# codyheiser/MILWRM

Hardware: AMD Instinct MI355X
Metric: pixels/sec (node) for preprocess+k-means fit+label, 30-ch MxIF k=8; %HBM peak (higher is better)
Workload: dtype f32 (fp64 accumulation)

## Files before the change

### include/milwrm_amd.h

```cpp
#ifndef MILWRM_AMD_H
#define MILWRM_AMD_H

#include <stddef.h>
#include <stdint.h>

#ifdef __cplusplus
extern "C" {
#endif

#define MW_OK 0
#define MW_EINVAL (-1)
#define MW_EHIP (-2)
#define MW_EUNSUPPORTED (-3)

#define MW_U8 0
#define MW_U16 1
#define MW_F32 2

int mw_version(void);
const char* mw_last_error(void);
int mw_stream_blocks(int64_t n);
int64_t mw_rows_per_block(int64_t n);

size_t mw_nz_stats_ws_bytes(int64_t n_pix, int C);
// ... 39 lines not shown
                     void* d_ws, void* stream);
size_t mw_image_moments_rows_ws_bytes(int64_t slide_H);
int mw_image_moments_rows(const void* d_img, int dtype, int H, int W, int C,
                          int64_t row_off, int64_t slide_H, int pass,
                          const float* d_inv_mean, float pseudoval, void* d_ws, void* stream);
int mw_image_moments_rows_final(int64_t slide_H, int W, int C, int with_m2,
                                void* d_ws, double* d_out, void* stream);

size_t mw_blur_ws_bytes(int H, int W, int C, int radius);
int mw_blur(const void* d_img, int dtype, int H, int W, int C,
            const float* d_inv_mean, float pseudoval,
            const float* h_w, int radius, float* d_out, void* d_ws, void* stream);

int mw_block_mean(const void* d_img, int dtype, int H, int W, int C, int fact,
                  float* d_out, void* stream);

size_t mw_mask_rank_ws_bytes(int64_t n_pix);
int mw_mask_rank(const uint8_t* d_mask, int64_t n_pix, uint32_t* d_rank2pix,
                 int64_t* d_count, void* d_ws, void* stream);

size_t mw_rank_index_bytes(int64_t n_pix);
int mw_mask_rank_index(const uint8_t* d_mask, int64_t n_pix, void* d_index, int64_t* d_count, void* d_ws,
                       void* stream);

size_t mw_gather_ws_bytes(int64_t S, int F);
int mw_gather_rows(const float* d_img, int C, const int32_t* d_feat, int F,
                   const int32_t* d_idx, const uint32_t* d_rank2pix, int64_t S,
                   float* d_X, void* d_ws, void* stream);
int mw_gather_rows_ri(const float* d_img, int C, const int32_t* d_feat, int F, const int32_t* d_idx,
                      const void* d_index, int64_t n_pix, int64_t pix_off, int64_t S, float* d_X, void* d_ws,
                      void* stream);
int mw_rank_to_pixel_ri(int32_t* d_idx, int64_t S, const void* d_index, int64_t n_pix, int64_t pix_off,
                        void* stream);
int mw_gather_rows_px(const float* d_img, int C, const int32_t* d_feat, int F, const int32_t* d_pix, int64_t S,
                      float* d_X, void* d_ws, void* stream);
int mw_col_stats_rows(const float* d_X, int64_t S, int F, void* d_ws, void* stream);

size_t mw_sample_slot_elems(int64_t n_pix);
int mw_sample_map(const int32_t* d_idx, const uint32_t* d_rank2pix, int64_t S, int64_t n_pix,
                  int32_t* d_slots, int32_t* d_ovf, void* stream);
int mw_blur_sample(const void* d_img, int dtype, int H, int W, int C, const float* d_inv_mean,
                   float pseudoval, const float* h_weights, int radius, const int32_t* d_slots,
                   int64_t S, const int32_t* d_feat, int F, float* d_X, void* stream);
int mw_sample_overflow(const int32_t* d_idx, const uint32_t* d_rank2pix, const int32_t* d_slots,
                       const int32_t* d_ovf, int64_t S, int F, float* d_X, void* stream);
int mw_sample_map_ri(const int32_t* d_idx, const void* d_index, int64_t n_index, int64_t pix_off, int64_t S,
// ... 199 lines not shown
```

### milwrm_amd/MILWRM.py

```python
from __future__ import annotations

import itertools
import os

import numpy as np
import pandas as pd
import torch

from . import _native as N
from . import device as D
from .assign import (DOM_REC, assign_image, assign_rows, banded_assign_image, blur_assign_image,
                     dm_total, dom_carry_, dom_sums, domain_means, domain_sse_deferred, domain_sse_image,
                     domain_sse_rows, LabelPassQC)
from .kmeans import DeviceRows, KMeans, StandardScaler, fit_many
from .MxIF import checktype, img
from .ST import blur_features_st
from .dist import LOCAL_COMM
from .rng import _release_last_draw, check_total, set_global_state_after_draws, subsample_indices_device
from .stream import band_filter



def kMeansRes(scaled_data, k, alpha_k=0.02, random_state=18, comm=None):
    comm = LOCAL_COMM if comm is None else comm
# ... 205 lines not shown
                                      image._mask_device(), out_rows=out_rows, qc=q)
        if res is None and how != "fused" and fusable:
            res = blur_assign_image(raw, sigma, inv_mean, p, mu, inv, centers, image._mask_device(),
                                    truncate=truncate)
            q = None
        if res is not None:
            return out(res)
    elif image._pending_median is not None or image._pending_bilateral is not None:
        res = banded_assign_image(image._source() or image._device(), band_filter(image), feats, mu, inv,
                                  centers, image._mask_device(), qc=q)
        if res is not None:
            return out(res)
    src = D.as_float32(image._materialize())
    if band is not None:
        return out(assign_image(src[band.rows], feats, mu, inv, centers,
                                D.padded_mask(image._mask_device()[band.rows].contiguous())))
    res = assign_image(src, feats, mu, inv, centers, image._mask_device())
    if q is not None:
        q.band(src, res[0])
    return out(res)


_SIDE = {}
GATHER_BY_PIXEL = os.environ.get("MW_GATHER_PX", "0") == "1"
DRAWS_BESIDE = os.environ.get("MW_DRAWS_BESIDE", "1") != "0"


def _draws_beside(M: int, fract: float, dev, after: torch.cuda.Event, index=None):
    main = torch.cuda.current_stream(dev)
    side = _SIDE.get(str(dev))
    if side is None:
        side = _SIDE[str(dev)] = torch.cuda.Stream(device=dev)
    side.wait_event(after)
    with torch.cuda.stream(side):
        idx, tot = subsample_indices_device(M, fract, 16, dev)
        if index is not None:
            D.rank_to_pixel(idx, index)
    main.wait_stream(side)
    idx.record_stream(main)
    tot.record_stream(main)
    return idx, tot


def _gather_deferred(image: img, feat, idx, r2p, X_out) -> bool:
    from .stream import bilateral_gather, blur_gather, median_gather

    if image._pending_median is not None:
        inv_mean, p = image._pending if image._pending is not None else (None, 1.0)
        return median_gather(image._source() or image._device(), image._pending_median, inv_mean, p, feat,
                             idx, r2p, X_out)
    if image._pending_bilateral is not None:
        inv_mean, p = image._pending if image._pending is not None else (None, 1.0)
        return bilateral_gather(image._source() or image._device(), image._pending_bilateral, inv_mean, p, feat,
                                idx, r2p, X_out)
    if image._pending_blur is None:
        return False
    sigma, truncate = image._pending_blur
    inv_mean, p = image._pending
    return blur_gather(image._source() or image._device(), sigma, inv_mean, p, feat, idx, r2p, X_out,
                       truncate=truncate)
# ... 199 lines not shown
            if filter_kwargs is not None:
                raise NotImplementedError("filter_kwargs on a slide in row bands: the banded pass "
                                          "runs the gaussian only")
            X, img_stats, xmax = prep_banded(images[0], self.image_df["batch_names"].iloc[0],
                                             means, features, filter_name, sigma, fract, comm)
            self._batch_counts = [int(X.shape[0])]
            self._images = images
            st = comm.merge_image_stats(D.d2h(img_stats), X.shape[1])
            self.scaler = StandardScaler.from_stats(st)
            mu, inv = self.scaler.affine()
            self._rows = DeviceRows(X, mu, inv, feature_var=self.scaler.var_ * inv * inv,
                                    xmax_local=D.d2h(xmax))
            self._cluster_host = None
            return
        batches = list(self.image_df["batch_names"])
        ev0 = torch.cuda.Event()
        ev0.record()
        if images:
            images[0].log_normalize(mean=means[batches[0]])
            images[0].blurring(filter_name=filter_name, sigma=sigma, **fkw)
        dev = D.device()
        ranks = []
        for i, im in enumerate(images):
            r2p, M = im._mask_rank()
            ranks.append((r2p if i == 0 else None, M))
        counts = [int(M * fract) for _, M in ranks]
        F = len(images[0]._features(features))
        _check_rows_fit(sum(counts), F, dev)
        X = torch.empty((sum(counts), F), dtype=torch.float32, device=dev)
        img_stats = torch.zeros((len(images), 1 + 2 * F), dtype=torch.float64, device=dev)
        xmax = torch.zeros(F, dtype=torch.float32, device=dev)
        def by_pixel(im, r2p):
            return isinstance(r2p, D.RankIndex) and not im._filter_deferred() and GATHER_BY_PIXEL

        pre = None
        if images and counts[0] and DRAWS_BESIDE and not images[0]._filter_deferred():
            px0 = by_pixel(images[0], ranks[0][0])
            pre = _draws_beside(ranks[0][1], fract, dev, ev0, ranks[0][0] if px0 else None) + (px0,)
        off = 0
        paths = []
        totals = []
        draws = []
        moments = []
        rank_base = 0
        for n_img, (im, batch, (r2p, M), S) in enumerate(
                zip(images, self.image_df["batch_names"], ranks, counts)):
            if n_img > 0:
                im.log_normalize(mean=means[batch])
                im.blurring(filter_name=filter_name, sigma=sigma, **fkw)
            np.random.seed(16)
            if S:
                if r2p is None:
                    r2p, _ = im._mask_rank()
                if n_img == 0 and pre is not None:
                    idx, tot, px = pre
                    pre = None
                else:
                    idx, tot = subsample_indices_device(M, fract, 16, dev)
                    px = by_pixel(im, r2p)
                    if px:
                        D.rank_to_pixel(idx, r2p)
                totals.append((tot, S))
                feat = D.h2d(np.asarray(im._features(features), dtype=np.int32), dev)
                if _gather_deferred(im, feat, idx, r2p, X[off:off + S]):
                    rec = D.col_stats_rows(X[off:off + S], img_stats[n_img], accumulate=False,
                                           absmax=xmax, keep_records=True)
                else:
                    rec = D.gather_rows(D.as_float32(im._materialize()), feat, idx, None if px else r2p,
                                        X[off:off + S], img_stats[n_img], accumulate=False, absmax=xmax,
                                        keep_records=True)
                moments.append((off, S) + rec)
                draws.append((off, S, idx, rank_base))
                del idx
            else:
                _release_last_draw()
            r2p = None
            ranks[n_img] = (None, M)
            off += S
            rank_base += int(im.shape[0]) * int(im.shape[1])
            if use_path:
                paths.append(_save_preprocessed(im, self.image_df["Img"].iloc[n_img], path_save))
        self._batch_counts = counts
        if use_path:
            self.image_df["Img"] = paths
        else:
            self._images = images
        set_global_state_after_draws()
        host = D.d2h(img_stats, xmax, *[t for t, _ in totals])
        for (_, S), tot in zip(totals, host[2:]):
            check_total(int(tot[0]), S)
        st = comm.merge_image_stats(host[0], F)
# ... 274 lines not shown
```

### milwrm_amd/MxIF.py

```python
from __future__ import annotations

import os

import numpy as np
import torch

from . import device as D
from .rng import check_total, set_global_state_after_draws, subsample_indices_device


def checktype(obj):
    return bool(obj) and all(isinstance(elem, str) for elem in obj)


def _out_of_scope(name):
    def f(*a, **k):
        raise NotImplementedError(f"{name} is outside the MI355X hot path (plotting); use the reference "
                                  "implementation")
    f.__name__ = name
    return f


def _need_kernel_size(name):
    return NotImplementedError(f"{name}: pass kernel_size= (an int, a (rows, cols) pair, or None for an eighth "
# ... 300 lines not shown
        return (self._pending_blur is not None or self._pending_median is not None
                or self._pending_bilateral is not None)

    @property
    def mask(self):
        return self._mask

    @mask.setter
    def mask(self, m):
        self._mask = m
        self._mask_dev = None
        self._mrank = None

    def _mask_device(self) -> torch.Tensor:
        if self._mask_dev is None:
            if self._mask is None:
                raise AssertionError("No tissue mask available")
            m = np.ascontiguousarray(np.asarray(self._mask) != 0, dtype=np.uint8)
            self._mask_dev = D.padded_mask(torch.from_numpy(m).to(D.device()))
        return self._mask_dev

    def _prefetch_mask_rank(self):
        if getattr(self, "_mrank", None) is None and self._mask is not None:
            self._mrank = D.mask_rank_async(self._mask_device().reshape(-1))

    def _mask_rank(self):
        pending = getattr(self, "_mrank", None)
        self._mrank = None
        return D.mask_rank(self._mask_device().reshape(-1), pending)

    def __repr__(self) -> str:
        descr = "img object with {} of {} and shape {}px x {}px\n".format(
            np.ndarray, np.dtype("float64"), self.shape[0], self.shape[1]
        ) + "{} image channels:\n\t{}".format(self.n_ch, self.ch)
        if self.mask is not None:
            descr += "\n\ntissue mask {} of {} and shape {}px x {}px".format(
                type(self.mask), self.mask.dtype, self.mask.shape[0], self.mask.shape[1])
        return descr

    def copy(self) -> "img":
        new = img.__new__(img)
        new.__dict__.update(self.__dict__)
        new.ch = list(self.ch)
        new._host = None if self._host is None else self._host.copy()
        new._host64 = None if self._host64 is None else self._host64.copy()
        new._dev = None if self._dev is None else self._dev.clone()
        new._hsrc = None
        new._mask = None if self._mask is None else self._mask.copy()
        new._mask_dev = None
        new._mrank = None
        return new

# ... 341 lines not shown
            print("mean calculated to perform log normalization")
            s, _ = self._nz_stats()
            n = self.shape[0] * self.shape[1]
            mean = s.cpu().numpy() / n
        elif self._pending is not None or self._pending_blur is not None or self._pending_bilateral is not None:
            self._materialize()
        mean = np.asarray(mean, dtype=np.float64)
        with np.errstate(divide="ignore"):
            inv = (1.0 / mean).astype(np.float32)
        raw = self._raw_int_max() is not None and self._pending is None and self._pending_blur is None
        self._pending = (D.h2d(inv, D.device()), float(pseudoval))
        self._lognorm_host = (inv, float(pseudoval)) if raw else None
        self._xbound = None
        self._host64 = None

    def _subsample_device(self, features, fract=0.2, random_state=16, X_out=None, stats=None,
                          accumulate=False):
        from .stream import bilateral_gather, blur_gather, median_gather

        features = self._features(features)
        np.random.seed(random_state)
        deferred = self._filter_deferred()
        src = None if deferred else D.as_float32(self._materialize())
        r2p, M = self._mask_rank()
        dev = D.device()
        d_idx, total = subsample_indices_device(M, fract, random_state, dev)
        S = d_idx.shape[0]
        if X_out is None:
            X_out = torch.empty((S, len(features)), dtype=torch.float32, device=dev)
        if stats is None:
            stats = torch.zeros(1 + 2 * len(features), dtype=torch.float64, device=dev)
        if S:
            feat = D.h2d(np.asarray(features, dtype=np.int32), dev)
            if deferred:
                inv, p = self._pending if self._pending is not None else (None, 1.0)
                if self._pending_median is not None:
                    median_gather(self._source() or self._device(), self._pending_median, inv, p, feat,
                                  d_idx, r2p, X_out)
                elif self._pending_bilateral is not None:
                    bilateral_gather(self._source() or self._device(), self._pending_bilateral, inv, p, feat,
                                     d_idx, r2p, X_out)
                else:
                    sigma, truncate = self._pending_blur
                    blur_gather(self._source() or self._device(), sigma, inv, p, feat, d_idx, r2p, X_out,
                                truncate)
                D.col_stats_rows(X_out, stats, accumulate)
            else:
# ... 76 lines not shown
```

### milwrm_amd/_native.py

```python
from __future__ import annotations

import ctypes as C
import os
import threading

import torch

_HERE = os.path.dirname(os.path.abspath(__file__))
LIB_PATH = os.environ.get("MW_LIB") or os.path.join(_HERE, "libmilwrm_amd.so")

MW_U8, MW_U16, MW_F32 = 0, 1, 2
_EINVAL, _EHIP, _EUNSUP = -1, -2, -3

_lib = None
_lock = threading.Lock()

c_i64, c_i32, c_u32, c_u64 = C.c_int64, C.c_int, C.c_uint32, C.c_uint64
c_f32, c_sz, c_vp = C.c_float, C.c_size_t, C.c_void_p
c_dp = C.POINTER(C.c_double)

_PROTOS = {
    "mw_version": (c_i32, []),
    "mw_host_labels_f64": (c_i32, [c_vp, c_i64, c_vp, c_i32]),
    "mw_host_f32_to_f64": (c_i32, [c_vp, c_i64, c_vp, c_i32]),
# ... 91 lines not shown
    "mw_domain_sse": (c_i32, [c_vp, c_i32, c_vp, c_i32, c_vp, c_vp, c_vp, c_vp, c_vp, c_i32, c_i32, c_vp,
                              c_i64, c_vp, c_i32, c_vp, c_vp]),
    "mw_domain_sse_f64": (c_i32, [c_vp, c_i32, c_vp, c_i32, c_vp, c_vp, c_vp, c_vp, c_vp, c_i32, c_i32, c_vp,
                                  c_i64, c_vp, c_i32, c_vp, c_vp]),
    "mw_neighbor_mean": (c_i32, [c_vp, c_vp, c_i64, c_vp, c_i32, c_vp, c_vp]),
    "mw_col_stats_rows": (c_i32, [c_vp, c_i64, c_i32, c_vp, c_vp]),
    "mw_col_stats_absmax": (c_i32, [c_vp, c_i64, c_i32, c_vp, c_i32, c_vp]),
    "mw_sample_slot_elems": (c_sz, [c_i64]),
    "mw_sample_map": (c_i32, [c_vp, c_vp, c_i64, c_i64, c_vp, c_vp, c_vp]),
    "mw_blur_sample": (c_i32, [c_vp, c_i32, c_i32, c_i32, c_i32, c_vp, c_f32, c_vp, c_i32, c_vp, c_i64, c_vp, c_i32, c_vp, c_vp]),
    "mw_sample_overflow": (c_i32, [c_vp, c_vp, c_vp, c_vp, c_i64, c_i32, c_vp, c_vp]),
    "mw_blur_assign_conf": (c_i32, [c_vp, c_i32, c_i32, c_i32, c_i32, c_vp, c_f32, c_vp, c_i32, c_vp, c_vp, c_vp, c_i32, c_vp, c_vp, c_vp, c_vp]),
    "mw_domain_records": (c_i32, [c_vp, c_vp, c_i64, c_i32, c_i32, c_vp, c_vp]),
    "mw_synth_slide": (c_i32, [c_i32, c_i32, c_i32, c_vp, c_i32, c_vp, c_i32, c_i32, c_i32, c_u64, c_vp, c_vp, c_vp]),
    "mw_synth_rows": (c_i32, [c_i32, c_i32, c_i32, c_i32, c_i32, c_vp, c_i32, c_vp, c_i32, c_i32, c_i32, c_u64,
                              c_vp, c_vp, c_vp]),
    "mw_blur_sample_rows": (c_i32, [c_vp, c_i32, c_i32, c_i32, c_i32, c_i64, c_i32, c_i32, c_vp, c_f32, c_vp,
                                    c_i32, c_vp, c_i64, c_vp, c_i32, c_vp, c_vp]),
    "mw_rank_index_bytes": (c_sz, [c_i64]),
    "mw_mask_rank_index": (c_i32, [c_vp, c_i64, c_vp, c_vp, c_vp, c_vp]),
    "mw_gather_rows_ri": (c_i32, [c_vp, c_i32, c_vp, c_i32, c_vp, c_vp, c_i64, c_i64, c_i64, c_vp, c_vp, c_vp]),
    "mw_rank_to_pixel_ri": (c_i32, [c_vp, c_i64, c_vp, c_i64, c_i64, c_vp]),
    "mw_gather_rows_px": (c_i32, [c_vp, c_i32, c_vp, c_i32, c_vp, c_i64, c_vp, c_vp, c_vp]),
    "mw_sample_map_ri": (c_i32, [c_vp, c_vp, c_i64, c_i64, c_i64, c_i64, c_vp, c_vp, c_vp]),
    "mw_sample_overflow_ri": (c_i32, [c_vp, c_vp, c_i64, c_i64, c_vp, c_vp, c_i64, c_i32, c_vp, c_vp]),
    "mw_slot_gather": (c_i32, [c_vp, c_i32, c_i64, c_i64, c_vp, c_i64, c_vp, c_i32, c_vp, c_vp]),
    "mw_blur_assign_rows": (c_i32, [c_vp, c_i32, c_i32, c_i32, c_i32, c_i64, c_i32, c_i32, c_vp, c_f32, c_vp,
                                    c_i32, c_vp, c_vp, c_vp, c_i32, c_vp, c_vp, c_vp, c_vp]),
}

EXPORTED = tuple(_PROTOS)


class LloydFit(C.Structure):
    _fields_ = [("centers", c_vp), ("drift", c_vp), ("half_sep", c_vp), ("labels", c_vp),
                ("ub", c_vp), ("lb", c_vp), ("ws", c_vp), ("out", c_vp), ("k", c_i32),
                ("drift_max", c_f32), ("inertia_exp", c_i32)]


class KppSeg(C.Structure):
    _fields_ = [("row_start", c_i64), ("n_rows", c_i64), ("rows_per_block", c_i64), ("d_records", c_vp)]


ALL_REDUCE_SUM_FN = C.CFUNCTYPE(c_i32, c_vp, c_i64, c_i64, c_vp)
ALL_GATHER_FN = C.CFUNCTYPE(c_i32, c_vp, c_i64, c_i64, c_i64, c_vp)

# ... 62 lines not shown
```

### milwrm_amd/csrc/preprocess.hip

```cpp
#include <stdarg.h>
#include <math.h>

#include "common.h"
#include "blur.h"

namespace mw {

static thread_local char g_err[512];

void set_error(const char* fmt, ...) {
  va_list ap;
  va_start(ap, fmt);
  vsnprintf(g_err, sizeof(g_err), fmt, ap);
  va_end(ap);
}

constexpr int kTile = 256;
constexpr int kMaxBlocks = 1024;

static inline int stream_blocks(int64_t n) {
  int64_t tiles = (n + kTile - 1) / kTile;
  if (tiles < 1) tiles = 1;
  return (int)(tiles < kMaxBlocks ? tiles : kMaxBlocks);
}
// ... 288 lines not shown

__global__ void __launch_bounds__(256) mask_count_kernel(const uint8_t* __restrict__ m, int64_t n,
                                                         uint32_t* __restrict__ cnt) {
  __shared__ uint32_t s_red[4];
  const int64_t lo = (int64_t)blockIdx.x * kMaskChunk;
  uint32_t c = 0;
  for (int it = 0; it < kMaskChunk / 4096; ++it) {
    const int64_t p = lo + (int64_t)it * 4096 + threadIdx.x * 16;
    if (p + 16 <= n) {
      uint4 v = *reinterpret_cast<const uint4*>(m + p);
      const uint32_t w[4] = {v.x, v.y, v.z, v.w};
#pragma unroll
      for (int k = 0; k < 4; ++k)
#pragma unroll
        for (int b = 0; b < 4; ++b) c += ((w[k] >> (8 * b)) & 0xFF) ? 1u : 0u;
    } else {
      for (int64_t q = p; q < n && q < p + 16; ++q) c += m[q] ? 1u : 0u;
    }
  }
  const uint32_t tot = block_sum(c, s_red);
  if (threadIdx.x == 0) cnt[blockIdx.x] = tot;
}

__global__ void __launch_bounds__(1024) mask_scan_kernel(uint32_t* __restrict__ cnt, int nb,
                                                         int64_t* __restrict__ count) {
  __shared__ unsigned long long s[1024];
  const int t = threadIdx.x;
  const int per = (nb + 1023) / 1024;
  const int lo = t * per, hi = min(nb, lo + per);
  unsigned long long loc = 0;
  for (int i = lo; i < hi; ++i) loc += cnt[i];
  s[t] = loc;
  __syncthreads();
  for (int o = 1; o < 1024; o <<= 1) {
    unsigned long long v = t >= o ? s[t - o] : 0ull;
    __syncthreads();
    s[t] += v;
    __syncthreads();
  }
  unsigned long long run = s[t] - loc;
  for (int i = lo; i < hi; ++i) {
    const uint32_t c = cnt[i];
    cnt[i] = (uint32_t)run;
    run += c;
  }
  if (t == 1023) *count = (int64_t)s[1023];
}

struct RankIndexPtrs {
  const uint64_t* bits;
  const uint32_t* pre;
  const uint32_t* blk;
};
__host__ __device__ inline int64_t rank_words(int64_t n) { return (n + 63) / 64; }
__host__ __device__ inline size_t rank_al(size_t x) { return (x + 255) & ~(size_t)255; }
__host__ __device__ inline size_t rank_pre_off(int64_t n) { return rank_al((size_t)rank_words(n) * 8); }
__host__ __device__ inline size_t rank_blk_off(int64_t n) {
  return rank_pre_off(n) + rank_al((size_t)(rank_words(n) + 1) * 4);
}
__host__ __device__ inline size_t rank_index_bytes(int64_t n) {
  return rank_blk_off(n) + rank_al((size_t)(rank_words(n) + 1) * 4);
}
__host__ __device__ inline RankIndexPtrs rank_ptrs(const void* base, int64_t n) {
  const char* b = reinterpret_cast<const char*>(base);
  return RankIndexPtrs{reinterpret_cast<const uint64_t*>(b), reinterpret_cast<const uint32_t*>(b + rank_pre_off(n)),
                       reinterpret_cast<const uint32_t*>(b + rank_blk_off(n))};
}
__device__ __forceinline__ uint32_t select64(uint64_t m, uint32_t r) {
  uint32_t pos = 0;
// ... 96 lines not shown
    }
    const uint32_t c = __popc(bits);
    uint32_t incl = c;
#pragma unroll
    for (int o = 1; o < 64; o <<= 1) {
      const uint32_t v = __shfl_up(incl, o, 64);
      if (lane >= o) incl += v;
    }
    if (lane == 63) s_w[wid] = incl;
    __syncthreads();
    uint32_t wbase = 0;
    for (int w = 0; w < wid; ++w) wbase += s_w[w];
    uint32_t loc = wbase + incl - c;
    while (bits) {
      const int q = __ffs(bits) - 1;
      bits &= bits - 1;
      s_pix[loc++] = (uint32_t)(p + q);
    }
    const uint32_t tot = s_w[0] + s_w[1] + s_w[2] + s_w[3];
    __syncthreads();
    for (uint32_t i = t; i < tot; i += 256) r2p[run + i] = s_pix[i];
    run += tot;
    __syncthreads();
  }
}

__device__ __forceinline__ void chan_merge(double& n_a, double& m_a, double& q_a, double n_b,
                                           double m_b, double q_b) {
  if (n_b == 0.0) return;
  if (n_a == 0.0) { n_a = n_b; m_a = m_b; q_a = q_b; return; }
  const double n = n_a + n_b;
  const double d = m_b - m_a;
  m_a += d * (n_b / n);
  q_a += q_b + d * d * (n_a * n_b / n);
  n_a = n;
}

template <bool GATHER, bool RI = false, bool PX = false>
__global__ void __launch_bounds__(256) gather_kernel(const float* __restrict__ img, int C,
                                                     const int32_t* __restrict__ feat, int F,
                                                     const int32_t* __restrict__ idx,
                                                     const uint32_t* __restrict__ r2p, int64_t S,
                                                     int64_t R, float* __restrict__ X,
                                                     double* __restrict__ rec, RankIndexPtrs ix = {},
                                                     int64_t pix_off = 0) {
  auto pix_of = [&](int32_t rho) -> uint32_t {
// ... 379 lines not shown
  }
}

int mw_block_mean(const void* d_img, int dtype, int H, int W, int C, int fact, float* d_out,
                  void* stream) {
  MW_CHECK_ARG(d_img && d_out, "mw_block_mean: null pointer");
  MW_CHECK_ARG(H > 0 && W > 0 && C > 0 && fact > 0, "mw_block_mean: bad shape");
  const int Ho = (H + fact - 1) / fact, Wo = (W + fact - 1) / fact;
  const int64_t n = (int64_t)Ho * Wo * C;
  const int grid = (int)std::min<int64_t>((n + 255) / 256, 8192);
  hipStream_t st = as_stream(stream);
  switch (dtype) {
    case MW_U8: hipLaunchKernelGGL(block_mean_kernel<uint8_t>, dim3(grid), dim3(256), 0, st, (const uint8_t*)d_img, H, W, C, fact, Ho, Wo, d_out); break;
    case MW_U16: hipLaunchKernelGGL(block_mean_kernel<uint16_t>, dim3(grid), dim3(256), 0, st, (const uint16_t*)d_img, H, W, C, fact, Ho, Wo, d_out); break;
    case MW_F32: hipLaunchKernelGGL(block_mean_kernel<float>, dim3(grid), dim3(256), 0, st, (const float*)d_img, H, W, C, fact, Ho, Wo, d_out); break;
    default: set_error("mw_block_mean: bad dtype %d", dtype); return MW_EINVAL;
  }
  MW_LAUNCH_CHECK();
  return MW_OK;
}

size_t mw_mask_rank_ws_bytes(int64_t n_pix) {
  const int64_t nb = (n_pix + kMaskChunk - 1) / kMaskChunk;
  return (size_t)nb * sizeof(uint32_t) + 256;
}

int mw_mask_rank(const uint8_t* d_mask, int64_t n_pix, uint32_t* d_rank2pix, int64_t* d_count,
                 void* d_ws, void* stream) {
  MW_CHECK_ARG(d_mask && d_rank2pix && d_count && d_ws, "mw_mask_rank: null pointer");
  MW_CHECK_ARG(n_pix > 0 && n_pix < (int64_t)4294967295LL, "mw_mask_rank: n_pix out of range");
  MW_CHECK_ARG(((uintptr_t)d_mask & 15) == 0, "mw_mask_rank: mask must be 16-byte aligned");
  hipStream_t st = as_stream(stream);
  const int nb = (int)((n_pix + kMaskChunk - 1) / kMaskChunk);
  uint32_t* cnt = reinterpret_cast<uint32_t*>(d_ws);
  hipLaunchKernelGGL(mask_count_kernel, dim3(nb), dim3(256), 0, st, d_mask, n_pix, cnt);
  MW_LAUNCH_CHECK();
  hipLaunchKernelGGL(mask_scan_kernel, dim3(1), dim3(1024), 0, st, cnt, nb, d_count);
  MW_LAUNCH_CHECK();
  hipLaunchKernelGGL(mask_scatter_kernel, dim3(nb), dim3(256), 0, st, d_mask, n_pix, cnt, d_rank2pix);
  MW_LAUNCH_CHECK();
  return MW_OK;
}

size_t mw_rank_index_bytes(int64_t n_pix) { return rank_index_bytes(n_pix); }

int mw_mask_rank_index(const uint8_t* d_mask, int64_t n_pix, void* d_index, int64_t* d_count, void* d_ws,
                       void* stream) {
  MW_CHECK_ARG(d_mask && d_index && d_count && d_ws, "mw_mask_rank_index: null pointer");
  MW_CHECK_ARG(n_pix > 0 && n_pix < (int64_t)4294967295LL - 64, "mw_mask_rank_index: n_pix out of range");
  MW_CHECK_ARG(((uintptr_t)d_mask & 15) == 0, "mw_mask_rank_index: mask must be 16-byte aligned");
  hipStream_t st = as_stream(stream);
  const int nb = (int)((n_pix + kMaskChunk - 1) / kMaskChunk);
  uint32_t* cnt = reinterpret_cast<uint32_t*>(d_ws);
  hipLaunchKernelGGL(mask_count_kernel, dim3(nb), dim3(256), 0, st, d_mask, n_pix, cnt);
  MW_LAUNCH_CHECK();
  hipLaunchKernelGGL(mask_scan_kernel, dim3(1), dim3(1024), 0, st, cnt, nb, d_count);
  MW_LAUNCH_CHECK();
  char* b = reinterpret_cast<char*>(d_index);
  hipLaunchKernelGGL(rank_words_kernel, dim3(nb), dim3(256), 0, st, d_mask, n_pix, cnt, d_count,
                     reinterpret_cast<uint64_t*>(b), reinterpret_cast<uint32_t*>(b + rank_pre_off(n_pix)),
                     reinterpret_cast<uint32_t*>(b + rank_blk_off(n_pix)));
  MW_LAUNCH_CHECK();
  return MW_OK;
}

int mw_gather_rows_ri(const float* d_img, int C, const int32_t* d_feat, int F, const int32_t* d_idx,
                      const void* d_index, int64_t n_pix, int64_t pix_off, int64_t S, float* d_X, void* d_ws,
                      void* stream) {
  MW_CHECK_ARG(d_img && d_feat && d_idx && d_index && d_X && d_ws, "mw_gather_rows_ri: null pointer");
  MW_CHECK_ARG(S > 0 && F > 0 && F <= 64 && C > 0 && n_pix > 0 && pix_off >= 0,
               "mw_gather_rows_ri: bad shape S=%lld F=%d", (long long)S, F);
  hipStream_t st = as_stream(stream);
  const int G = stream_blocks(S);
  const int64_t R = rows_per_block(S);
  size_t lds = (size_t)kTile * F * sizeof(float);
  if (lds < 4 * 256 * sizeof(double)) lds = 4 * 256 * sizeof(double);
  hipLaunchKernelGGL((gather_kernel<true, true>), dim3(G), dim3(256), lds, st, d_img, C, d_feat, F, d_idx,
                     nullptr, S, R, d_X, reinterpret_cast<double*>(d_ws), rank_ptrs(d_index, n_pix), pix_off);
  MW_LAUNCH_CHECK();
  return MW_OK;
}

__global__ void __launch_bounds__(256) rank_to_pixel_kernel(int32_t* __restrict__ idx, int64_t S,
                                                            RankIndexPtrs ix, int64_t pix_off) {
// ... 332 lines not shown
```

### milwrm_amd/device.py

```python
from __future__ import annotations

import os

import numpy as np
import torch

from . import _native as N
from . import profiling

_DTYPE_CODE = {torch.uint8: N.MW_U8, torch.int16: N.MW_U16, torch.float32: N.MW_F32}


def require_gpu():
    if not torch.cuda.is_available():
        raise RuntimeError("milwrm_amd runs on an AMD Instinct GPU (HIP); no device is visible "
                           "and there is no CPU fallback")
    N.load()


def device():
    require_gpu()
    return torch.device("cuda", torch.cuda.current_device())


# ... 497 lines not shown
    return out


def block_mean(img: torch.Tensor, fact: int):
    H, W, C = img.shape
    Ho, Wo = -(-H // fact), -(-W // fact)
    out = torch.empty((Ho, Wo, C), dtype=torch.float32, device=img.device)
    N.call("mw_block_mean", P(img), dtype_code(img), H, W, C, int(fact), P(out), stream())
    return out


class RankIndex:

    def __init__(self, buf: torch.Tensor, n_pix: int, pix_off: int = 0):
        self.buf, self.n_pix, self.pix_off = buf, int(n_pix), int(pix_off)

    def offset(self, k: int) -> "RankIndex":
        return RankIndex(self.buf, self.n_pix, self.pix_off + int(k))

    def __getitem__(self, sl):
        return self


_RT = os.environ.get("MW_RANK_TABLE")
RANK_TABLE_MAX_PIX = (1 << 62) if _RT == "1" else 0 if _RT == "0" else (1 << 28)


def mask_rank_async(mask_u8: torch.Tensor):
    n = mask_u8.numel()
    cnt = torch.empty(1, dtype=torch.int64, device=mask_u8.device)
    ws = WS.get("mrank", N.query("mw_mask_rank_ws_bytes", n))
    if n <= RANK_TABLE_MAX_PIX:
        r2p = torch.empty(n, dtype=torch.int32, device=mask_u8.device)
        with profiling.timed("mask_rank", n):
            N.call("mw_mask_rank", P(mask_u8), n, P(r2p), P(cnt), P(ws), stream())
    else:
        buf = torch.empty(N.query("mw_rank_index_bytes", n), dtype=torch.uint8, device=mask_u8.device)
        with profiling.timed("mask_rank", n):
            N.call("mw_mask_rank_index", P(mask_u8), n, P(buf), P(cnt), P(ws), stream())
        r2p = RankIndex(buf, n)
    slot = _PINNED.take(8)
    slot[1] = _Busy
    hv = slot[0][:8].view(torch.int64)
    hv.copy_(cnt, non_blocking=True)
    ev = torch.cuda.Event()
    ev.record()
    return r2p, cnt, (slot, hv, ev)


def mask_rank(mask_u8: torch.Tensor, pending=None):
    r2p, cnt, (slot, hv, ev) = mask_rank_async(mask_u8) if pending is None else pending
    ev.synchronize()
    M = int(hv[0])
    slot[1] = None
    return r2p[:M], M


def gather_rows(img_f32: torch.Tensor, feat: torch.Tensor, idx: torch.Tensor, r2p: torch.Tensor,
                X_out: torch.Tensor, stats: torch.Tensor, accumulate: bool, absmax=None,
                keep_records=False):
    H, W, C = img_f32.shape
    S, F = X_out.shape
    if S == 0:
        return None
    ws = _records_ws(S, F, keep_records, X_out.device)
    with profiling.timed("gather", S * (F * 4 * 2 + 8)):
        if r2p is None:
            N.call("mw_gather_rows_px", P(img_f32), C, P(feat), F, P(idx), S, P(X_out), P(ws), stream())
        elif isinstance(r2p, RankIndex):
            N.call("mw_gather_rows_ri", P(img_f32), C, P(feat), F, P(idx), P(r2p.buf), r2p.n_pix, r2p.pix_off,
                   S, P(X_out), P(ws), stream())
        else:
            N.call("mw_gather_rows", P(img_f32), C, P(feat), F, P(idx), P(r2p), S, P(X_out), P(ws),
                   stream())
    N.call("mw_col_stats_finalize", P(ws), S, F, P(stats), 1 if accumulate else 0, stream())
    if absmax is not None:
        N.call("mw_col_stats_absmax", P(ws), S, F, P(absmax), 1, stream())
    return (N.query("mw_rows_per_block", S), ws) if keep_records else None


def _records_ws(S: int, F: int, keep: bool, dev):
    nb = N.query("mw_gather_ws_bytes", S, F)
    return torch.empty(nb, dtype=torch.uint8, device=dev) if keep else WS.get("gather", nb)


def rank_to_pixel(idx: torch.Tensor, index: "RankIndex"):
    S = idx.numel()
    if S:
        with profiling.timed("rank_to_pixel", S * 8):
            N.call("mw_rank_to_pixel_ri", P(idx), S, P(index.buf), index.n_pix, index.pix_off, stream())
    return idx


def col_stats_rows(X: torch.Tensor, stats: torch.Tensor, accumulate: bool, absmax=None,
                   keep_records=False):
    S, F = X.shape
    if S == 0:
        return None
    ws = _records_ws(S, F, keep_records, X.device)
    with profiling.timed("col_stats", S * F * 4):
        N.call("mw_col_stats_rows", P(X), S, F, P(ws), stream())
    N.call("mw_col_stats_finalize", P(ws), S, F, P(stats), 1 if accumulate else 0, stream())
    if absmax is not None:
        N.call("mw_col_stats_absmax", P(ws), S, F, P(absmax), 1, stream())
    return (N.query("mw_rows_per_block", S), ws) if keep_records else None


FUSED_USED = {"sample": 0, "assign": 0, "assign_banded": 0, "sample_streamed": 0, "assign_streamed": 0,
              "nz_streamed": 0}
MEDIAN_USED = {"network": 0, "generic": 0, "rows_streamed": 0}
BILATERAL_USED = {"rows_streamed": 0}


# ... 39 lines not shown
```

Baseline: 6.433 billion.

## Replace mask rank table with run-length index plus binary-search rank-to-pixel

Adds a run-length encoded mask rank index: one kernel counts set pixels and run starts per chunk, a scan kernel computes offsets, a third writes (rank, pixel) run pairs, and a fourth builds a coarse top-level lookup table. Sampled ranks are turned into pixel indices by a shared-memory-bucketed binary search over the runs. Gathering then uses the direct-pixel path. This avoids writing and reading a full per-pixel int32 rank table, at the cost of an extra pass over the mask, a search per sample, and a fallback to the old path when the number of runs exceeds the cap.

```diff
diff --git a/include/milwrm_amd.h b/include/milwrm_amd.h
--- a/include/milwrm_amd.h
+++ b/include/milwrm_amd.h
@@ -85,6 +85,12 @@
 size_t mw_rank_index_bytes(int64_t n_pix);
 int mw_mask_rank_index(const uint8_t* d_mask, int64_t n_pix, void* d_index, int64_t* d_count, void* d_ws,
                        void* stream);
+
+size_t mw_mask_rank_runs_bytes(int64_t nr_max);
+int mw_mask_rank_runs(const uint8_t* d_mask, int64_t n_pix, void* d_runs, int64_t nr_max, int64_t* d_count,
+                      void* d_ws, void* stream);
+int mw_rank_to_pixel_runs(int32_t* d_idx, int64_t S, const void* d_runs, int64_t n_pix, int64_t pix_off,
+                          void* stream);
 
 size_t mw_gather_ws_bytes(int64_t S, int F);
 int mw_gather_rows(const float* d_img, int C, const int32_t* d_feat, int F,
diff --git a/milwrm_amd/MILWRM.py b/milwrm_amd/MILWRM.py
--- a/milwrm_amd/MILWRM.py
+++ b/milwrm_amd/MILWRM.py
@@ -251,11 +251,10 @@
 
 
 _SIDE = {}
-GATHER_BY_PIXEL = os.environ.get("MW_GATHER_PX", "0") == "1"
 DRAWS_BESIDE = os.environ.get("MW_DRAWS_BESIDE", "1") != "0"
 
 
-def _draws_beside(M: int, fract: float, dev, after: torch.cuda.Event, index=None):
+def _draws_beside(M: int, fract: float, dev, after: torch.cuda.Event):
     main = torch.cuda.current_stream(dev)
     side = _SIDE.get(str(dev))
     if side is None:
@@ -263,8 +262,6 @@
     side.wait_event(after)
     with torch.cuda.stream(side):
         idx, tot = subsample_indices_device(M, fract, 16, dev)
-        if index is not None:
-            D.rank_to_pixel(idx, index)
     main.wait_stream(side)
     idx.record_stream(main)
     tot.record_stream(main)
@@ -510,7 +507,7 @@
         dev = D.device()
         ranks = []
         for i, im in enumerate(images):
-            r2p, M = im._mask_rank()
+            r2p, M = im._mask_rank(runs=i > 0 or not im._filter_deferred())
             ranks.append((r2p if i == 0 else None, M))
         counts = [int(M * fract) for _, M in ranks]
         F = len(images[0]._features(features))
@@ -518,13 +515,9 @@
         X = torch.empty((sum(counts), F), dtype=torch.float32, device=dev)
         img_stats = torch.zeros((len(images), 1 + 2 * F), dtype=torch.float64, device=dev)
         xmax = torch.zeros(F, dtype=torch.float32, device=dev)
-        def by_pixel(im, r2p):
-            return isinstance(r2p, D.RankIndex) and not im._filter_deferred() and GATHER_BY_PIXEL
-
         pre = None
         if images and counts[0] and DRAWS_BESIDE and not images[0]._filter_deferred():
-            px0 = by_pixel(images[0], ranks[0][0])
-            pre = _draws_beside(ranks[0][1], fract, dev, ev0, ranks[0][0] if px0 else None) + (px0,)
+            pre = _draws_beside(ranks[0][1], fract, dev, ev0)
         off = 0
         paths = []
         totals = []
@@ -539,22 +532,19 @@
             np.random.seed(16)
             if S:
                 if r2p is None:
-                    r2p, _ = im._mask_rank()
+                    r2p, _ = im._mask_rank(runs=not im._filter_deferred())
                 if n_img == 0 and pre is not None:
-                    idx, tot, px = pre
+                    idx, tot = pre
                     pre = None
                 else:
                     idx, tot = subsample_indices_device(M, fract, 16, dev)
-                    px = by_pixel(im, r2p)
-                    if px:
-                        D.rank_to_pixel(idx, r2p)
                 totals.append((tot, S))
                 feat = D.h2d(np.asarray(im._features(features), dtype=np.int32), dev)
                 if _gather_deferred(im, feat, idx, r2p, X[off:off + S]):
                     rec = D.col_stats_rows(X[off:off + S], img_stats[n_img], accumulate=False,
                                            absmax=xmax, keep_records=True)
                 else:
-                    rec = D.gather_rows(D.as_float32(im._materialize()), feat, idx, None if px else r2p,
+                    rec = D.gather_rows(D.as_float32(im._materialize()), feat, idx, r2p,
                                         X[off:off + S], img_stats[n_img], accumulate=False, absmax=xmax,
                                         keep_records=True)
                 moments.append((off, S) + rec)
diff --git a/milwrm_amd/MxIF.py b/milwrm_amd/MxIF.py
--- a/milwrm_amd/MxIF.py
+++ b/milwrm_amd/MxIF.py
@@ -346,12 +346,13 @@
 
     def _prefetch_mask_rank(self):
         if getattr(self, "_mrank", None) is None and self._mask is not None:
-            self._mrank = D.mask_rank_async(self._mask_device().reshape(-1))
-
-    def _mask_rank(self):
+            runs = not self._filter_deferred() and self._source() is None
+            self._mrank = D.mask_rank_async(self._mask_device().reshape(-1), runs)
+
+    def _mask_rank(self, runs=False):
         pending = getattr(self, "_mrank", None)
         self._mrank = None
-        return D.mask_rank(self._mask_device().reshape(-1), pending)
+        return D.mask_rank(self._mask_device().reshape(-1), pending, runs)
 
     def __repr__(self) -> str:
         descr = "img object with {} of {} and shape {}px x {}px\n".format(
@@ -739,7 +740,7 @@
         np.random.seed(random_state)
         deferred = self._filter_deferred()
         src = None if deferred else D.as_float32(self._materialize())
-        r2p, M = self._mask_rank()
+        r2p, M = self._mask_rank(runs=not deferred)
         dev = D.device()
         d_idx, total = subsample_indices_device(M, fract, random_state, dev)
         S = d_idx.shape[0]
diff --git a/milwrm_amd/_native.py b/milwrm_amd/_native.py
--- a/milwrm_amd/_native.py
+++ b/milwrm_amd/_native.py
@@ -137,6 +137,9 @@
     "mw_gather_rows_ri": (c_i32, [c_vp, c_i32, c_vp, c_i32, c_vp, c_vp, c_i64, c_i64, c_i64, c_vp, c_vp, c_vp]),
     "mw_rank_to_pixel_ri": (c_i32, [c_vp, c_i64, c_vp, c_i64, c_i64, c_vp]),
     "mw_gather_rows_px": (c_i32, [c_vp, c_i32, c_vp, c_i32, c_vp, c_i64, c_vp, c_vp, c_vp]),
+    "mw_mask_rank_runs_bytes": (c_sz, [c_i64]),
+    "mw_mask_rank_runs": (c_i32, [c_vp, c_i64, c_vp, c_i64, c_vp, c_vp, c_vp]),
+    "mw_rank_to_pixel_runs": (c_i32, [c_vp, c_i64, c_vp, c_i64, c_i64, c_vp]),
     "mw_sample_map_ri": (c_i32, [c_vp, c_vp, c_i64, c_i64, c_i64, c_i64, c_vp, c_vp, c_vp]),
     "mw_sample_overflow_ri": (c_i32, [c_vp, c_vp, c_i64, c_i64, c_vp, c_vp, c_i64, c_i32, c_vp, c_vp]),
     "mw_slot_gather": (c_i32, [c_vp, c_i32, c_i64, c_i64, c_vp, c_i64, c_vp, c_i32, c_vp, c_vp]),
diff --git a/milwrm_amd/csrc/preprocess.hip b/milwrm_amd/csrc/preprocess.hip
--- a/milwrm_amd/csrc/preprocess.hip
+++ b/milwrm_amd/csrc/preprocess.hip
@@ -334,9 +334,8 @@
   if (threadIdx.x == 0) cnt[blockIdx.x] = tot;
 }
 
-__global__ void __launch_bounds__(1024) mask_scan_kernel(uint32_t* __restrict__ cnt, int nb,
-                                                         int64_t* __restrict__ count) {
-  __shared__ unsigned long long s[1024];
+__device__ __forceinline__ unsigned long long mask_scan_block(uint32_t* __restrict__ cnt, int nb,
+                                                              unsigned long long* s) {
   const int t = threadIdx.x;
   const int per = (nb + 1023) / 1024;
   const int lo = t * per, hi = min(nb, lo + per);
@@ -356,7 +355,16 @@
     cnt[i] = (uint32_t)run;
     run += c;
   }
-  if (t == 1023) *count = (int64_t)s[1023];
+  const unsigned long long tot = s[1023];
+  __syncthreads();
+  return tot;
+}
+
+__global__ void __launch_bounds__(1024) mask_scan_kernel(uint32_t* __restrict__ cnt, int nb,
+                                                         int64_t* __restrict__ count) {
+  __shared__ unsigned long long s[1024];
+  const unsigned long long tot = mask_scan_block(cnt, nb, s);
+  if (threadIdx.x == 1023) *count = (int64_t)tot;
 }
 
 struct RankIndexPtrs {
@@ -499,6 +507,208 @@
     for (uint32_t i = t; i < tot; i += 256) r2p[run + i] = s_pix[i];
     run += tot;
     __syncthreads();
+  }
+}
+
+constexpr int kRunTop = 8191;
+enum { kRunHdrMagic = 0, kRunHdrCount = 1, kRunHdrOverflow = 2 };
+struct RunIndexPtrs {
+  uint32_t* hdr;
+  uint32_t* top;
+  uint2* run;
+};
+__host__ __device__ inline size_t run_top_off() { return 256; }
+__host__ __device__ inline size_t run_pairs_off() { return run_top_off() + rank_al((size_t)(kRunTop + 1) * 4); }
+__host__ __device__ inline size_t run_index_bytes(int64_t nr_max) {
+  return run_pairs_off() + rank_al((size_t)(nr_max + 1) * 8);
+}
+inline RunIndexPtrs run_ptrs(const void* base) {
+  char* b = const_cast<char*>(reinterpret_cast<const char*>(base));
+  return RunIndexPtrs{reinterpret_cast<uint32_t*>(b), reinterpret_cast<uint32_t*>(b + run_top_off()),
+                      reinterpret_cast<uint2*>(b + run_pairs_off())};
+}
+__device__ __forceinline__ uint32_t run_key(uint32_t rho, uint32_t magic) {
+  return min(__umulhi(rho, magic), (uint32_t)kRunTop - 1u);
+}
+
+__device__ __forceinline__ void mask_flags16(const uint8_t* __restrict__ m, int64_t n, int64_t p, int lane,
+                                             uint32_t& bits, uint32_t& starts) {
+  bits = 0;
+  if (p + 16 <= n) {
+    const uint4 v = *reinterpret_cast<const uint4*>(m + p);
+    const uint32_t w[4] = {v.x, v.y, v.z, v.w};
+#pragma unroll
+    for (int k = 0; k < 4; ++k)
+#pragma unroll
+      for (int q = 0; q < 4; ++q) bits |= ((w[k] >> (8 * q)) & 0xFFu) ? 1u << (4 * k + q) : 0u;
+  } else {
+    for (int q = 0; q < 16; ++q)
+      if (p + q < n && m[p + q]) bits |= 1u << q;
+  }
+  uint32_t prev = __shfl_up(bits >> 15, 1, 64);
+  if (lane == 0) prev = (p > 0 && p - 1 < n && m[p - 1]) ? 1u : 0u;
+  starts = bits & ~((bits << 1) | prev) & 0xFFFFu;
+}
+
+__global__ void __launch_bounds__(256) mask_count_runs_kernel(const uint8_t* __restrict__ m, int64_t n,
+                                                              uint32_t* __restrict__ cnt,
+                                                              uint32_t* __restrict__ rcnt) {
+  __shared__ uint32_t s_red[4];
+  const int64_t lo = (int64_t)blockIdx.x * kMaskChunk;
+  uint32_t c = 0;
+  for (int it = 0; it < kMaskChunk / 4096; ++it) {
+    uint32_t bits, starts;
+    mask_flags16(m, n, lo + (int64_t)it * 4096 + threadIdx.x * 16, threadIdx.x & 63, bits, starts);
+    c += __popc(bits) | (__popc(starts) << 16);
+  }
+  const uint32_t tot = block_sum(c, s_red);
+  if (threadIdx.x == 0) {
+    cnt[blockIdx.x] = tot & 0xFFFFu;
+    rcnt[blockIdx.x] = tot >> 16;
+  }
+}
+
+__global__ void __launch_bounds__(1024) mask_scan_runs_kernel(uint32_t* __restrict__ cnt,
+                                                              uint32_t* __restrict__ rcnt, int nb,
+                                                              int64_t nr_max, int64_t* __restrict__ count,
+                                                              RunIndexPtrs rx) {
+  __shared__ unsigned long long s[1024];
+  const unsigned long long M = mask_scan_block(cnt, nb, s);
+  const unsigned long long nr = mask_scan_block(rcnt, nb, s);
+  if (threadIdx.x == 0) {
+    const bool over = nr > (unsigned long long)nr_max;
+    count[0] = (int64_t)M;
+    count[1] = (int64_t)nr;
+    count[2] = over ? 1 : 0;
+    const unsigned long long mg = M ? ((unsigned long long)kRunTop << 32) / M : 0xFFFFFFFFull;
+    rx.hdr[kRunHdrMagic] = (uint32_t)(mg < 0xFFFFFFFFull ? mg : 0xFFFFFFFFull);
+    rx.hdr[kRunHdrCount] = over ? 0u : (uint32_t)nr;
+    rx.hdr[kRunHdrOverflow] = over ? 1u : 0u;
+    if (!over) rx.run[nr] = make_uint2((uint32_t)M, 0u);
+  }
+}
+
+__global__ void __launch_bounds__(256) mask_runs_kernel(const uint8_t* __restrict__ m, int64_t n,
+                                                        const uint32_t* __restrict__ base,
+                                                        const uint32_t* __restrict__ rbase,
+                                                        const int64_t* __restrict__ count, int64_t nr_max,
+                                                        RunIndexPtrs rx) {
+  __shared__ uint32_t s_w[4];
+  if (count[2]) return;
+  const int t = threadIdx.x, lane = t & 63, wid = t >> 6;
+  uint32_t ri = rbase[blockIdx.x];
+  const uint32_t re = blockIdx.x + 1 < gridDim.x ? rbase[blockIdx.x + 1] : (uint32_t)count[1];
+  if (ri == re) return;
+  uint32_t run = base[blockIdx.x];
+  const int64_t lo = (int64_t)blockIdx.x * kMaskChunk;
+  for (int it = 0; it < kMaskChunk / 4096 && ri < re; ++it) {
+    const int64_t p = lo + (int64_t)it * 4096 + t * 16;
+    uint32_t bits, starts;
+    mask_flags16(m, n, p, lane, bits, starts);
+    const uint32_t c = __popc(bits) | (__popc(starts) << 16);
+    uint32_t incl = c;
+#pragma unroll
+    for (int o = 1; o < 64; o <<= 1) {
+      const uint32_t v = __shfl_up(incl, o, 64);
+      if (lane >= o) incl += v;
+    }
+    if (lane == 63) s_w[wid] = incl;
+    __syncthreads();
+    uint32_t excl = incl - c;
+    for (int w = 0; w < wid; ++w) excl += s_w[w];
+    uint32_t r = ri + (excl >> 16);
+    const uint32_t rk = run + (excl & 0xFFFFu);
+    while (starts) {
+      const int q = __ffs(starts) - 1;
+      starts &= starts - 1;
+      if ((int64_t)r < nr_max) rx.run[r] = make_uint2(rk + __popc(bits & ((1u << q) - 1u)), (uint32_t)(p + q));
+      ++r;
+    }
+    const uint32_t tot = s_w[0] + s_w[1] + s_w[2] + s_w[3];
+    run += tot & 0xFFFFu;
+    ri += tot >> 16;
+    __syncthreads();
+  }
+}
+
+__device__ __forceinline__ uint32_t run_search(const uint2* __restrict__ run, uint32_t lo, uint32_t hi,
+                                               uint32_t rho) {
+  while (lo < hi) {
+    const uint32_t mid = lo + ((hi - lo + 1) >> 1);
+    if (run[mid].x <= rho) lo = mid;
+    else hi = mid - 1;
+  }
+  return lo;
+}
+
+__global__ void __launch_bounds__(256) run_top_kernel(const int64_t* __restrict__ count, RunIndexPtrs rx) {
+  if (count[2]) return;
+  const uint32_t k = blockIdx.x * 256 + threadIdx.x;
+  if (k > (uint32_t)kRunTop) return;
+  const uint64_t M = (uint64_t)count[0];
+  const uint32_t nr = (uint32_t)count[1];
+  const uint64_t magic = rx.hdr[kRunHdrMagic];
+  const uint64_t r = (((uint64_t)k << 32) + magic - 1) / magic;
+  uint32_t i = nr ? nr - 1 : 0;
+  if (r < M) i = run_search(rx.run, 0, nr - 1, (uint32_t)r);
+  rx.top[k] = i;
+}
+
+__global__ void __launch_bounds__(256) rank_to_pixel_runs_kernel(int32_t* __restrict__ idx, int64_t S,
+                                                                 RunIndexPtrs rx, int64_t pix_off) {
+  __shared__ uint32_t s_top[kRunTop + 1];
+  if (rx.hdr[kRunHdrOverflow] || rx.hdr[kRunHdrCount] == 0) return;
+  for (int i = threadIdx.x; i <= kRunTop; i += 256) s_top[i] = rx.top[i];
+  const uint32_t magic = rx.hdr[kRunHdrMagic];
+  const uint2* __restrict__ run = rx.run;
+  __syncthreads();
+  constexpr int U = 4;
+  const int64_t stride = (int64_t)gridDim.x * 256;
+  for (int64_t j0 = (int64_t)blockIdx.x * 256 + threadIdx.x; j0 < S; j0 += U * stride) {
+    uint32_t rho[U], lo[U], hi[U];
+    uint2 cur[U];
+    bool have[U];
+    bool more = false;
+#pragma unroll
+    for (int u = 0; u < U; ++u) {
+      rho[u] = j0 + u * stride < S ? (uint32_t)idx[j0 + u * stride] : 0u;
+      const uint32_t k = run_key(rho[u], magic);
+      lo[u] = s_top[k];
+      hi[u] = s_top[k + 1];
+      have[u] = false;
+      more |= lo[u] < hi[u];
+    }
+    while (more) {
+      uint32_t mid[U];
+      uint2 v[U];
+#pragma unroll
+      for (int u = 0; u < U; ++u) {
+        mid[u] = lo[u] + ((hi[u] - lo[u] + 1) >> 1);
+        v[u] = run[lo[u] < hi[u] ? mid[u] : 0u];
+      }
+      more = false;
+#pragma unroll
+      for (int u = 0; u < U; ++u) {
+        if (lo[u] < hi[u]) {
+          if (v[u].x <= rho[u]) {
+            lo[u] = mid[u];
+            cur[u] = v[u];
+            have[u] = true;
+          } else {
+            hi[u] = mid[u] - 1;
+          }
+        }
+        more |= lo[u] < hi[u];
+      }
+    }
+#pragma unroll
+    for (int u = 0; u < U; ++u) {
+      const uint2 f = run[have[u] ? 0u : lo[u]];
+      if (!have[u]) cur[u] = f;
+    }
+#pragma unroll
+    for (int u = 0; u < U; ++u)
+      if (j0 + u * stride < S) idx[j0 + u * stride] = (int32_t)(cur[u].y + (rho[u] - cur[u].x) + (uint32_t)pix_off);
   }
 }
 
@@ -924,7 +1134,7 @@
 
 size_t mw_mask_rank_ws_bytes(int64_t n_pix) {
   const int64_t nb = (n_pix + kMaskChunk - 1) / kMaskChunk;
-  return (size_t)nb * sizeof(uint32_t) + 256;
+  return 2 * (size_t)nb * sizeof(uint32_t) + 256;
 }
 
 int mw_mask_rank(const uint8_t* d_mask, int64_t n_pix, uint32_t* d_rank2pix, int64_t* d_count,
@@ -962,6 +1172,44 @@
   hipLaunchKernelGGL(rank_words_kernel, dim3(nb), dim3(256), 0, st, d_mask, n_pix, cnt, d_count,
                      reinterpret_cast<uint64_t*>(b), reinterpret_cast<uint32_t*>(b + rank_pre_off(n_pix)),
                      reinterpret_cast<uint32_t*>(b + rank_blk_off(n_pix)));
+  MW_LAUNCH_CHECK();
+  return MW_OK;
+}
+
+size_t mw_mask_rank_runs_bytes(int64_t nr_max) { return nr_max > 0 ? run_index_bytes(nr_max) : 0; }
+
+int mw_mask_rank_runs(const uint8_t* d_mask, int64_t n_pix, void* d_runs, int64_t nr_max, int64_t* d_count,
+                      void* d_ws, void* stream) {
+  MW_CHECK_ARG(d_mask && d_runs && d_count && d_ws, "mw_mask_rank_runs: null pointer");
+  MW_CHECK_ARG(n_pix > 0 && n_pix < (int64_t)4294967295LL, "mw_mask_rank_runs: n_pix out of range");
+  MW_CHECK_ARG(nr_max > 0 && nr_max < (int64_t)0x7fffffffLL, "mw_mask_rank_runs: nr_max out of range");
+  MW_CHECK_ARG(((uintptr_t)d_mask & 15) == 0, "mw_mask_rank_runs: mask must be 16-byte aligned");
+  MW_CHECK_ARG(((uintptr_t)d_runs & 7) == 0, "mw_mask_rank_runs: index must be 8-byte aligned");
+  hipStream_t st = as_stream(stream);
+  const int nb = (int)((n_pix + kMaskChunk - 1) / kMaskChunk);
+  uint32_t* cnt = reinterpret_cast<uint32_t*>(d_ws);
+  uint32_t* rcnt = cnt + nb;
+  const RunIndexPtrs rx = run_ptrs(d_runs);
+  hipLaunchKernelGGL(mask_count_runs_kernel, dim3(nb), dim3(256), 0, st, d_mask, n_pix, cnt, rcnt);
+  MW_LAUNCH_CHECK();
+  hipLaunchKernelGGL(mask_scan_runs_kernel, dim3(1), dim3(1024), 0, st, cnt, rcnt, nb, nr_max, d_count, rx);
+  MW_LAUNCH_CHECK();
+  hipLaunchKernelGGL(mask_runs_kernel, dim3(nb), dim3(256), 0, st, d_mask, n_pix, cnt, rcnt, d_count, nr_max, rx);
+  MW_LAUNCH_CHECK();
+  hipLaunchKernelGGL(run_top_kernel, dim3((kRunTop + 1 + 255) / 256), dim3(256), 0, st, d_count, rx);
+  MW_LAUNCH_CHECK();
+  return MW_OK;
+}
+
+int mw_rank_to_pixel_runs(int32_t* d_idx, int64_t S, const void* d_runs, int64_t n_pix, int64_t pix_off,
+                          void* stream) {
+  MW_CHECK_ARG(d_idx && d_runs, "mw_rank_to_pixel_runs: null pointer");
+  MW_CHECK_ARG(S >= 0 && n_pix > 0 && pix_off >= 0 && n_pix + pix_off <= 0x7fffffffll,
+               "mw_rank_to_pixel_runs: bad sizes S=%lld n_pix=%lld", (long long)S, (long long)n_pix);
+  if (S == 0) return MW_OK;
+  const int grid = (int)std::min<int64_t>((S + 1023) / 1024, 1024);
+  hipLaunchKernelGGL(rank_to_pixel_runs_kernel, dim3(grid), dim3(256), 0, as_stream(stream), d_idx, S,
+                     run_ptrs(d_runs), pix_off);
   MW_LAUNCH_CHECK();
   return MW_OK;
 }
diff --git a/milwrm_amd/device.py b/milwrm_amd/device.py
--- a/milwrm_amd/device.py
+++ b/milwrm_amd/device.py
@@ -543,36 +543,75 @@
         return self
 
 
+class RankRuns:
+
+    def __init__(self, buf: torch.Tensor, n_pix: int, nr_max: int, pix_off: int = 0):
+        self.buf, self.n_pix, self.nr_max, self.pix_off = buf, int(n_pix), int(nr_max), int(pix_off)
+        self.nr = None
+
+    def offset(self, k: int) -> "RankRuns":
+        r = RankRuns(self.buf, self.n_pix, self.nr_max, self.pix_off + int(k))
+        r.nr = self.nr
+        return r
+
+    def __getitem__(self, sl):
+        return self
+
+
 _RT = os.environ.get("MW_RANK_TABLE")
 RANK_TABLE_MAX_PIX = (1 << 62) if _RT == "1" else 0 if _RT == "0" else (1 << 28)
-
-
-def mask_rank_async(mask_u8: torch.Tensor):
+RANK_RUNS_MAX = 1 << 18
+MASK_RANK_USED = {"runs": 0, "table": 0, "index": 0, "runs_overflow": 0}
+
+
+def mask_rank_async(mask_u8: torch.Tensor, runs: bool = False):
     n = mask_u8.numel()
-    cnt = torch.empty(1, dtype=torch.int64, device=mask_u8.device)
     ws = WS.get("mrank", N.query("mw_mask_rank_ws_bytes", n))
-    if n <= RANK_TABLE_MAX_PIX:
+    if runs and _RT is None and RANK_RUNS_MAX > 0 and n < (1 << 31):
+        nr_max = int(RANK_RUNS_MAX)
+        cnt = torch.empty(3, dtype=torch.int64, device=mask_u8.device)
+        buf = torch.empty(N.query("mw_mask_rank_runs_bytes", nr_max), dtype=torch.uint8, device=mask_u8.device)
+        with profiling.timed("mask_rank", n):
+            N.call("mw_mask_rank_runs", P(mask_u8), n, P(buf), nr_max, P(cnt), P(ws), stream())
+        r2p = RankRuns(buf, n, nr_max)
+        MASK_RANK_USED["runs"] += 1
+    elif n <= RANK_TABLE_MAX_PIX:
+        cnt = torch.empty(1, dtype=torch.int64, device=mask_u8.device)
         r2p = torch.empty(n, dtype=torch.int32, device=mask_u8.device)
         with profiling.timed("mask_rank", n):
             N.call("mw_mask_rank", P(mask_u8), n, P(r2p), P(cnt), P(ws), stream())
+        MASK_RANK_USED["table"] += 1
     else:
+        cnt = torch.empty(1, dtype=torch.int64, device=mask_u8.device)
         buf = torch.empty(N.query("mw_rank_index_bytes", n), dtype=torch.uint8, device=mask_u8.device)
         with profiling.timed("mask_rank", n):
             N.call("mw_mask_rank_index", P(mask_u8), n, P(buf), P(cnt), P(ws), stream())
         r2p = RankIndex(buf, n)
-    slot = _PINNED.take(8)
+        MASK_RANK_USED["index"] += 1
+    nb = 8 * cnt.numel()
+    slot = _PINNED.take(nb)
     slot[1] = _Busy
-    hv = slot[0][:8].view(torch.int64)
+    hv = slot[0][:nb].view(torch.int64)
     hv.copy_(cnt, non_blocking=True)
     ev = torch.cuda.Event()
     ev.record()
     return r2p, cnt, (slot, hv, ev)
 
 
-def mask_rank(mask_u8: torch.Tensor, pending=None):
-    r2p, cnt, (slot, hv, ev) = mask_rank_async(mask_u8) if pending is None else pending
+def mask_rank(mask_u8: torch.Tensor, pending=None, runs: bool = False):
+    if pending is not None and isinstance(pending[0], RankRuns) and not runs:
+        pending[2][2].synchronize()
+        pending[2][0][1] = None
+        pending = None
+    r2p, cnt, (slot, hv, ev) = mask_rank_async(mask_u8, runs) if pending is None else pending
     ev.synchronize()
     M = int(hv[0])
+    if isinstance(r2p, RankRuns):
+        r2p.nr, over = int(hv[1]), int(hv[2])
+        if over:
+            slot[1] = None
+            MASK_RANK_USED["runs_overflow"] += 1
+            return mask_rank(mask_u8)
     slot[1] = None
     return r2p[:M], M
 
@@ -585,6 +624,9 @@
     if S == 0:
         return None
     ws = _records_ws(S, F, keep_records, X_out.device)
+    if isinstance(r2p, RankRuns):
+        rank_to_pixel(idx, r2p)
+        r2p = None
     with profiling.timed("gather", S * (F * 4 * 2 + 8)):
         if r2p is None:
             N.call("mw_gather_rows_px", P(img_f32), C, P(feat), F, P(idx), S, P(X_out), P(ws), stream())
@@ -605,11 +647,16 @@
     return torch.empty(nb, dtype=torch.uint8, device=dev) if keep else WS.get("gather", nb)
 
 
-def rank_to_pixel(idx: torch.Tensor, index: "RankIndex"):
+def rank_to_pixel(idx: torch.Tensor, index):
     S = idx.numel()
     if S:
         with profiling.timed("rank_to_pixel", S * 8):
-            N.call("mw_rank_to_pixel_ri", P(idx), S, P(index.buf), index.n_pix, index.pix_off, stream())
+            if isinstance(index, RankRuns):
+                if index.nr is None or index.nr > index.nr_max:
+                    raise RuntimeError("rank_to_pixel: the run index is not complete (mask_rank checks it)")
+                N.call("mw_rank_to_pixel_runs", P(idx), S, P(index.buf), index.n_pix, index.pix_off, stream())
+            else:
+                N.call("mw_rank_to_pixel_ri", P(idx), S, P(index.buf), index.n_pix, index.pix_off, stream())
     return idx
 
 
```

Result: no change. 6.522 billion, median of 6 (+1.4%).
